# aask1357/hilcodec

Hardware: AMD Instinct MI355X
Metric: audio-seconds/sec (xRT) encode+RVQ+decode, 24 kHz batch=256 (higher is better)
Workload: dtype f32

## Files before the change

hilcodec_amd/csrc/resblock_cfg.h:

```cpp
#pragma once
#include <stdlib.h>

#include <atomic>
#include <type_traits>

#include "gemm_core.h"

using namespace hilc;

namespace {

constexpr int DWS = 12;

#ifndef HILC_RES_SHARE2_0
#define HILC_RES_SHARE2_0 0.61
#endif
#ifndef HILC_RES_SHARE3_0
#define HILC_RES_SHARE3_0 0.44
#define HILC_RES_SHARE3_1 0.31
#endif
template <int C, bool STREAM, bool SCARRY_ = false, int NB_ = 1, bool W8_ = false, int DR_ = 0, bool POST_ = false, bool SPEC0_ = false>
struct Cfg {
  static constexpr bool POST = POST_;
  static constexpr bool SPEC0 = SPEC0_;
  static_assert(!SPEC0_ || (C == 64 && (!STREAM || SCARRY_) && !W8_ && DR_ >= 0), "stage-0 input phase: the C = 64 encoder stage in the carry form (four waves, 128-column tiles)");
  static_assert(!POST_ || ((!STREAM || SCARRY_) && DR_ <= 0 && C <= 192 && !W8_), "closing conv: the carry form of a narrow stage (offline, or a hop's runs of whole streams)");
  static constexpr int NB = NB_;
  static constexpr int DR = DR_ > 0 ? DR_ : 0;
  static constexpr int UR = DR_ < 0 ? -DR_ : 0;
  static_assert(DR_ <= 0 || (((DR_ == 2 || DR_ == 4) && (!STREAM || SCARRY_) && C <= 192) || ((!STREAM || SCARRY_) && DR_ == 5 && C == 256) || (!SCARRY_ && DR_ == 8 && C == 512)),
                "down-sampling phase: carry form, r = 2 / 4 (C <= 192) or the wide encoder stages (C = 256: r = 5, offline and the hop's 32-column carry form; C = 512: r = 8, offline and a hop's whole-stream tiles)");
  static constexpr int DCAR = DR_ <= 0 ? 0 : (DR_ == 5 ? 12 : (DR_ == 8 ? 8 : 4));
  static_assert(DR_ >= 0 || ((DR_ == -8 && C >= 512) || (DR_ == -5 && C == 384) || ((DR_ == -4 || DR_ == -2) && C <= 192 && (!STREAM || SCARRY_))),
                "up-sampling phase: 32-column tiles (r = 8: whole streams, or the offline carry form), the C = 384 stage (r = 5) or the carry form (r = 4 / 2)");
  static constexpr int CH = C;
  static constexpr int CB = C / 32;
  static constexpr bool NARROW = C >= 256;
  static constexpr bool N32 = STREAM && SCARRY_ && NARROW;
  static_assert(!N32 || C == 256 || C == 384, "32-column carry form: the C = 256 / C = 384 stages of a hop");
  static constexpr int NCOL = NARROW ? ((C >= 512 || N32) ? 32 : 64) : 128;
  static constexpr int XS = NCOL + ((!STREAM || SCARRY_) ? 8 * NB_ + 2 * DCAR + (POST_ ? 4 : 0) : 0);
  static constexpr bool CARRYMODE = !STREAM || SCARRY_;
  static constexpr int HALO = CARRYMODE ? 0 : ((NARROW && C >= 512) ? 0 : 8);
  static constexpr int TO = NCOL - HALO;
  static constexpr int NW = (N32 && C == 384) ? 12 : ((C >= 192 || W8_) ? 8 : 4);
  static constexpr int NT = 64 * NW;
  static constexpr int RH = NW / (NCOL / 32);
  static constexpr int CBW = CB / RH;
  static constexpr int RPI = 256 / NCOL;
  static constexpr int RSTEP = RPI * NW;
  static constexpr int RW = C / RSTEP;
#ifndef HILC_RES_RB
#define HILC_RES_RB 4
#endif
  static constexpr int RB = HILC_RES_RB;
#ifdef HILC_RES_KP
  static constexpr int KP = HILC_RES_KP;
  static constexpr int DEPTH = HILC_RES_DEPTH;
#else
  static constexpr int KP = C >= 96 ? 4 : 8;
  static constexpr int DEPTH = C >= 256 ? 4 : (C == 128 ? (STREAM ? 2 : 3) : 2);
#endif
#ifndef HILC_RES_MINW
#define HILC_RES_MINW 2
#endif
  static constexpr int MINW = NW >= 8 ? NW / 4 : HILC_RES_MINW;
  static_assert(NW % (NCOL / 32) == 0 && CB % RH == 0 && RW % RB == 0 && C % RSTEP == 0, "tile split");
  static_assert(NB_ >= 1 && NB_ <= 3 && (NB_ == 1 || CARRYMODE || (NARROW && C >= 512)), "a chain needs carries or whole-stream tiles");
};

struct ResBlk {
  const float* w1t;
  const float* dw1_w;
  const float* dw1_b;
  const float* w2t;
  const float* dw2_w;
  const float* dw2_b;
  const float* hist1;
  const float* hist2;
  float* hist1_out;
  float* hist2_out;
  float pre_scale, out_scale;
};

struct ResUp {
  const float* xin;
  const float* tr_w;
  const float* w_lo;
  const float* w_hi;
  const float* bias;
  const float* hist;
  float* hist_out;
  float in_scale;
};

struct ResDown {
  const float* w_lo;
  const float* w_hi;
  const float* dw_w;
  const float* dw_b;
  const float* hist;
  float* hist_out;
  const float* res;
  float* y;
  float in_scale;
};

struct ResPost {
  const float* w;
  const float* bias;
  float* wav;
  const float* hist;
  float* hist_out;
  float in_scale, out_scale;
  int do_tanh;
};

struct ResSpec0 {
  const float* wav;
  const float* dft;
  const float* nyq;
  const float* pw;
  const float* bias;
  const float* pre_w;
  const float* pre_b;
  const float* hist;
  int hist_len;
  float pre_in_scale, mean, stdv, out_scale;
  int normalize;
};

constexpr int POST_CLASSES = 8;

constexpr int MAXBLK = 3;
constexpr int DDS = 12;

struct ResArgs {
  const float* x;
  ResBlk blk[MAXBLK];
  int nblk;
  ResDown dn;
  ResUp up;
  ResPost post;
  ResSpec0 spec;
  long run_tiles;
  float* y;
  int T, tiles;
  int classes;
  unsigned cum[5];
  long total_tiles;
  int B;
  unsigned div_magic, div_shift;
  int* sched;
  unsigned long long* dbg;
};

#ifdef HILC_DEBUG_STAMPS
unsigned long long* g_dbg = nullptr;
#endif

}
```

hilcodec_amd/csrc/resblock_gemm.h:

```cpp
#pragma once
#include "resblock_cfg.h"

namespace {

typedef const __attribute__((address_space(1))) float* gptr_t;
typedef __attribute__((address_space(3))) float* lptr_t;
typedef __attribute__((address_space(3))) f32x4* lvec_t;
typedef __attribute__((address_space(3))) f32x2* lvec2_t;

template <class K>
struct WeightPipe {
  static constexpr int CBW = K::CBW;
  static constexpr int DEPTH = K::DEPTH;
  static constexpr int KP = K::KP;
  static constexpr int WPS = KP * CBW / 4;
  static_assert(KP * CBW % 4 == 0 && 8 % KP == 0, "register set = whole 16-B words");
  float a[DEPTH][KP][CBW];
  __device__ __forceinline__ void load_word(gptr_t wset, int slot, int q, int lane) {
    typedef const __attribute__((address_space(1))) f32x4* gvec_t;
    const f32x4 v = *(gvec_t)(wset + q * 256 + lane * 4);
#pragma unroll
    for (int e = 0; e < 4; ++e) a[slot][(q * 4 + e) / CBW][(q * 4 + e) % CBW] = v[e];
  }
  __device__ __forceinline__ void prefetch(const float* __restrict__ wt, int lane) {
#pragma unroll
    for (int d = 0; d < DEPTH - 1; ++d)
#pragma unroll
      for (int q = 0; q < WPS; ++q) load_word((gptr_t)(wt + d * WPS * 256), d, q, lane);
  }
};


template <class K, bool ZERO = true>
__device__ __forceinline__ void gemm_phase(const float* __restrict__ wt, const float* X, f32x16 (&acc)[K::CBW],
                                           WeightPipe<K>& wp, int colblk, int lane) {
  constexpr int C = K::CH, XS = K::XS;
  constexpr int CBW = K::CBW;
  constexpr int DEPTH = WeightPipe<K>::DEPTH, KP = WeightPipe<K>::KP, WPS = WeightPipe<K>::WPS;
  constexpr int NSETS = C / 2 / KP;
  const int kh = lane >> 5, l31 = lane & 31;
  lptr_t xn = (lptr_t)(X + kh * XS + colblk * 32 + l31);
  float b[DEPTH][KP];
#pragma unroll
  for (int d = 0; d < DEPTH - 1; ++d) {
#pragma unroll
    for (int j = 0; j < KP; ++j) b[d][j] = xn[j * 2 * XS];
    xn += KP * 2 * XS;
    asm volatile("" : "+v"(xn));
  }
  constexpr int LD_EVERY = KP * CBW / WPS;
  const float* wn = wt + (DEPTH - 1) * WPS * 256;
#pragma unroll
  for (int s = 0; s < NSETS; ++s) {
    const int cur = s % DEPTH, nxt = (s + DEPTH - 1) % DEPTH;
    const int sn = s + DEPTH - 1;
    const bool more = sn < NSETS;
#pragma unroll
    for (int j = 0; j < KP; ++j) {
      if (more) b[nxt][j] = xn[j * 2 * XS];
#pragma unroll
      for (int i = 0; i < CBW; ++i) {
        const int n = j * CBW + i;
        if (more && n % LD_EVERY == 0) wp.load_word((gptr_t)wn, nxt, n / LD_EVERY, lane);
        if (ZERO && s == 0 && j == 0) {
#pragma unroll
          for (int r = 0; r < 16; ++r) acc[i][r] = 0.f;
        }
        acc[i] = __builtin_amdgcn_mfma_f32_32x32x2f32(wp.a[cur][j][i], b[cur][j], acc[i], 0, 0, 0);
      }
    }
    if (more) {
      xn += KP * 2 * XS;
      wn += WPS * 256;
      asm volatile("" : "+v"(xn), "+s"(wn));
    }
#pragma unroll
    for (int i = 0; i < CBW; ++i) asm volatile("" : "+v"(acc[i]) :: "memory");
  }
}

template <class K, bool ZERO = true>
__device__ __forceinline__ void gemm_phase_rolled(const float* __restrict__ wt, const float* X, f32x16 (&acc)[K::CBW],
                                                  WeightPipe<K>& wp, int colblk, int lane) {
  constexpr int C = K::CH, XS = K::XS;
  constexpr int CBW = K::CBW;
  constexpr int DEPTH = WeightPipe<K>::DEPTH, KP = WeightPipe<K>::KP, WPS = WeightPipe<K>::WPS;
  constexpr int NSETS = C / 2 / KP;
  static_assert(NSETS % DEPTH == 0 && NSETS >= 2 * DEPTH, "whole groups of register sets");
  constexpr int NG = NSETS / DEPTH;
  const int kh = lane >> 5, l31 = lane & 31;
  lptr_t xn = (lptr_t)(X + kh * XS + colblk * 32 + l31);
  float b[DEPTH][KP];
#pragma unroll
  for (int d = 0; d < DEPTH - 1; ++d) {
#pragma unroll
    for (int j = 0; j < KP; ++j) b[d][j] = xn[j * 2 * XS];
    xn += KP * 2 * XS;
    asm volatile("" : "+v"(xn));
  }
  constexpr int LD_EVERY = KP * CBW / WPS;
  const float* wn = wt + (DEPTH - 1) * WPS * 256;
  if constexpr (ZERO) {
#pragma unroll
    for (int i = 0; i < CBW; ++i)
#pragma unroll
      for (int r = 0; r < 16; ++r) acc[i][r] = 0.f;
  }
  auto one_set = [&](auto dc, bool more) {
    constexpr int cur = decltype(dc)::value, nxt = (cur + DEPTH - 1) % DEPTH;
#pragma unroll
    for (int j = 0; j < KP; ++j) {
      if (more) b[nxt][j] = xn[j * 2 * XS];
#pragma unroll
      for (int i = 0; i < CBW; ++i) {
        const int n = j * CBW + i;
        if (more && n % LD_EVERY == 0) wp.load_word((gptr_t)wn, nxt, n / LD_EVERY, lane);
        acc[i] = __builtin_amdgcn_mfma_f32_32x32x2f32(wp.a[cur][j][i], b[cur][j], acc[i], 0, 0, 0);
      }
    }
    if (more) {
      xn += KP * 2 * XS;
      wn += WPS * 256;
      asm volatile("" : "+v"(xn), "+s"(wn));
    }
#pragma unroll
    for (int i = 0; i < CBW; ++i) asm volatile("" : "+v"(acc[i]) :: "memory");
  };
  auto group = [&](bool last) {
    one_set(std::integral_constant<int, 0>{}, true);
    if constexpr (DEPTH > 1) one_set(std::integral_constant<int, 1>{}, !last);
    if constexpr (DEPTH > 2) one_set(std::integral_constant<int, 2>{}, !last);
    if constexpr (DEPTH > 3) one_set(std::integral_constant<int, 3>{}, !last);
    static_assert(DEPTH <= 4, "group body");
  };
#pragma nounroll
  for (int g = 0; g < NG - 1; ++g) group(false);
  group(true);
}

template <class K>
__device__ __forceinline__ void acc_to_x(const f32x16 (&acc)[K::CBW], float* X, int rowblk0, int colblk, int lane) {
  constexpr int XS = K::XS;
  lptr_t xb = (lptr_t)(X + (rowblk0 * 32 + 4 * (lane >> 5)) * XS + colblk * 32 + (lane & 31));
#pragma unroll
  for (int i = 0; i < K::CBW; ++i) {
#pragma unroll
    for (int r = 0; r < 16; ++r) xb[((r & 3) + 8 * (r >> 2)) * XS] = acc[i][r];
    xb += 32 * XS;
    asm volatile("" : "+v"(xb));
  }
}

__device__ __forceinline__ void lds_barrier() { asm volatile("s_waitcnt lgkmcnt(0)\n\ts_barrier" ::: "memory"); }

}
```

hilcodec_amd/csrc/resblock_kernel.h:

```cpp
#pragma once
#include "resblock_gemm.h"
#include "stream_gemm.h"

namespace {

struct Cols {
  long b;
  int t;
  int t_in;
  unsigned boff;
  unsigned hoff;
  int head, tail;
};
static_assert(sizeof(Cols) == 32, "no padding");

template <int C, bool STREAM, bool SCARRY = false, int NB = 1, bool W8 = false, int DRU = 0, bool POST = false, bool SPEC0 = false>
__global__ __launch_bounds__((Cfg<C, STREAM, SCARRY, NB, W8, DRU, POST, SPEC0>::NT), (Cfg<C, STREAM, SCARRY, NB, W8, DRU, POST, SPEC0>::MINW)) void resblock_kernel(ResArgs a) {
  using K = Cfg<C, STREAM, SCARRY, NB, W8, DRU, POST, SPEC0>;
  constexpr int DR = K::DR, UR = K::UR;
  using Pipe = WeightPipe<K>;
  constexpr int CBW = K::CBW, NW = K::NW, NT = K::NT, RW = K::RW, RB = K::RB, XS = K::XS, TO = K::TO, RSTEP = K::RSTEP;
  __shared__ __attribute__((aligned(16))) float Xbuf[4 + C * XS];
  constexpr bool DW_RELOAD = NB > 1 && K::NARROW && (4 + C * XS + NB * C * DWS) * 4 > 156 * 1024;
  __shared__ __attribute__((aligned(16))) float DW[(DW_RELOAD ? 1 : NB) * C * DWS];
// ... 106 lines not shown
          if (C % NT == 0 || m < C) {
#pragma unroll
            for (int w4 = 0; w4 < DWS / 4; ++w4)
              *reinterpret_cast<f32x4*>(&DW[(q * C + m) * DWS + 4 * w4]) =
                  f32x4{tv[q][it][4 * w4], tv[q][it][4 * w4 + 1], tv[q][it][4 * w4 + 2], tv[q][it][4 * w4 + 3]};
          }
        }
      }
    }
    }
  }
  if constexpr (DR > 0 && !DWIDE) {
    constexpr int RND = (2 * C + NT - 1) / NT;
    float tw[RND][2 * DR + 1];
#pragma unroll
    for (int it = 0; it < RND; ++it) {
      const int m = tid + it * NT;
      const int mc = ((2 * C) % NT == 0 || m < 2 * C) ? m : 2 * C - 1;
#pragma unroll
      for (int j = 0; j < 2 * DR; ++j) tw[it][j] = a.dn.dw_w[mc * 2 * DR + j];
      tw[it][2 * DR] = a.dn.dw_b[mc];
    }
#pragma unroll
    for (int it = 0; it < RND; ++it) {
      const int m = tid + it * NT;
      if ((2 * C) % NT == 0 || m < 2 * C) {
#pragma unroll
        for (int j = 0; j < DDS; ++j) DWD[m * DDS + j] = j < 2 * DR ? tw[it][j] : (j == 8 ? tw[it][2 * DR] : 0.f);
      }
    }
  }
  if (tid < 4) Xbuf[tid] = 0.f;
  const int rsub = wave * K::RPI + (K::RPI > 1 ? lane / (K::NCOL / 4) : 0);
  const int c4 = (lane & (K::NCOL / 4 - 1)) * 4;
  [[maybe_unused]] const unsigned row_b = (unsigned)T * 4u;
  [[maybe_unused]] const bool one_head = STREAM && !K::NARROW && T >= K::NCOL;

  auto columns_of = [&](long tile) -> Cols {
    Cols s;
    s.boff = 0; s.hoff = 0; s.head = false; s.tail = false;
    if constexpr (STREAM) {
      const int flat = (int)tile * TO - K::HALO + c4;
      s.t_in = flat >= 0 && flat < a.B * T;
      const unsigned ub = s.t_in ? __umulhi((unsigned)flat, a.div_magic) >> a.div_shift : 0u;
      s.b = ub;
      s.t = s.t_in ? flat - (int)ub * T : 0;
      s.boff = (ub * (unsigned)(C * T) + (unsigned)s.t) * 4u;
      s.hoff = ub * (unsigned)(C * 4);
      s.head = s.t_in && s.t == 0;
      s.tail = s.t_in && c4 >= K::HALO && s.t == T - 4;
    } else {
      s.b = tile / a.tiles;
      s.t = (int)(tile - s.b * a.tiles) * TO + c4;
      s.t_in = s.t >= 0 && s.t < T;
    }
    return s;
  };
  auto xrow = [&](const Cols& s, int m) -> const f32x4* {
    if constexpr (STREAM)
      return reinterpret_cast<const f32x4*>(reinterpret_cast<const char*>(a.x) + (s.boff + (unsigned)m * row_b));
    else
      return reinterpret_cast<const f32x4*>(a.x + s.b * (long)C * T + (long)m * T + (s.t_in ? s.t : 0));
  };
  auto yrow = [&](const Cols& s, int m) -> f32x4* {
    if constexpr (STREAM)
      return reinterpret_cast<f32x4*>(reinterpret_cast<char*>(a.y) + (s.boff + (unsigned)m * row_b));
    else
      return reinterpret_cast<f32x4*>(a.y + s.b * (long)C * T + (long)m * T + s.t);
  };

  [[maybe_unused]] const float* hb0 = a.x;
  [[maybe_unused]] const float* hb1 = a.x;
  [[maybe_unused]] bool hv0 = false, hv1 = false;
  [[maybe_unused]] int blk_off = 0;
  Cols cs;
  const bool lane0 = c4 == 0, lane_last = c4 == K::NCOL - 4;
  auto prev_base = [&](int which) -> lptr_t {
    if constexpr (!K::CARRYMODE) return (lptr_t)(X + rsub * XS + c4 - 4);
    else return lane0 ? (lptr_t)(X + rsub * XS + K::NCOL + which * 4 + blk_off) : (lptr_t)(X + rsub * XS + c4 - 4);
  };
  auto prevs_of = [&](lptr_t pb, int m0, int which, f32x4 (&prev)[K::RB]) {
    if constexpr (!STREAM) {
#pragma unroll
      for (int i = 0; i < K::RB; ++i) prev[i] = *(lvec_t)(pb + i * RSTEP * XS);
    } else {
      bool staged = false;
      if constexpr (!K::NARROW) staged = one_head;
      if (staged) {
#pragma unroll
        for (int i = 0; i < K::RB; ++i) {
          const lptr_t pa = cs.head ? (lptr_t)(HS + (which * C + m0 + RSTEP * i) * 4) : pb + i * RSTEP * XS;
          prev[i] = *(lvec_t)pa;
        }
      } else {
        f32x4 hv[K::RB];
#pragma unroll
        for (int i = 0; i < K::RB; ++i)
          hv[i] = *reinterpret_cast<const f32x4*>((which ? hb1 : hb0) + ((which ? hv1 : hv0) ? cs.hoff + (unsigned)(m0 + RSTEP * i) * 4u : 0u));
#pragma unroll
        for (int i = 0; i < K::RB; ++i) {
          const f32x4 own = *(lvec_t)(pb + i * RSTEP * XS);
#pragma unroll
          for (int e = 0; e < 4; ++e) prev[i][e] = cs.head ? ((which ? hv1 : hv0) ? hv[i][e] : 0.f) : own[e];
        }
      }
    }
  };
  auto carry_out = [&](lptr_t xp, int which, const f32x4 (&cur)[K::RB]) {
    if constexpr (K::CARRYMODE) {
      if (lane_last) {
#pragma unroll
        for (int i = 0; i < K::RB; ++i) *(lvec_t)(xp + i * RSTEP * XS + 4 + which * 4 + blk_off) = cur[i];
      }
    }
  };

  float touch = 0.f;
  constexpr int LPR = K::NCOL / 32;
#ifdef HILC_RES_NO_UTOUCH
  constexpr bool UTOUCH = false;
#else
  constexpr bool UTOUCH = !STREAM && UR > 0 && !K::NARROW && (K::NCOL / (UR > 0 ? UR : 1)) % 32 == 0;
#endif
  constexpr int LPRU = UTOUCH ? K::NCOL / UR / 32 : 1;
  constexpr int NTOUCH = STREAM ? 1 : (UTOUCH ? (2 * C * LPRU + NT - 1) / NT : (C * LPR + NT - 1) / NT);
  float tv[NTOUCH];
#pragma unroll
  for (int i = 0; i < NTOUCH; ++i) tv[i] = 0.f;
  __shared__ long s_next;
  long run0 = blockIdx.x, run1 = a.total_tiles;
  long tile = blockIdx.x;
  if constexpr (K::CARRYMODE) {
    if (a.classes > 1) {
      const unsigned P = gridDim.x / (unsigned)a.classes, u = blockIdx.x % P, c = blockIdx.x / P;
      const long s0 = (long)u * a.total_tiles / P, len = (long)(u + 1) * a.total_tiles / P - s0;
      run0 = s0 + ((len * (long)a.cum[c]) >> 16);
      run1 = s0 + ((len * (long)a.cum[c + 1]) >> 16);
    } else if (a.run_tiles > 0) {
      run0 = (long)blockIdx.x * a.run_tiles;
      run1 = run0 + a.run_tiles < a.total_tiles ? run0 + a.run_tiles : a.total_tiles;
    } else {
      run0 = (long)blockIdx.x * a.total_tiles / gridDim.x;
      run1 = ((long)blockIdx.x + 1) * a.total_tiles / gridDim.x;
    }
    const bool mid = STREAM ? (run0 * TO) % T != 0 : run0 % a.tiles != 0;
    tile = (mid && run0 < run1) ? run0 - 1 : run0;
  }
  cs = columns_of(tile < run1 ? tile : 0);
  f32x4 xr[RW];
  if (UR == 0 && !SPEC0 && tile < run1) {
#pragma unroll
    for (int i = 0; i < RW; ++i) xr[i] = *xrow(cs, rsub + RSTEP * i);
  }
  lds_barrier();
  while (tile < run1) {
    const bool warm = K::CARRYMODE && tile < run0;
    constexpr bool TICKETS = !K::CARRYMODE && K::NW == 4;
    if constexpr (K::CARRYMODE && !STREAM) {
      if (tile % a.tiles == 0) {
        constexpr int NSLOT = 2 * NB + K::DCAR / 2 + (POST ? 1 : 0);
        for (int e = tid; e < NSLOT * C; e += NT)
          *reinterpret_cast<f32x4*>(X + (e / NSLOT) * XS + K::NCOL + (e % NSLOT) * 4) = f32x4{0.f, 0.f, 0.f, 0.f};
      }
    }
    if constexpr (!K::CARRYMODE) {
      if (TICKETS && a.sched != nullptr && tid == 0) s_next = (long)gridDim.x + atomicAdd(a.sched, 1);
    }
#if defined(HILC_DEBUG_WAVE_STAMPS)
    if (a.dbg != nullptr) {
      if (ws_base != nullptr && lane == 0) ws_base[(WS_MAXB - 1) * 3 + 1] = (unsigned long long)ws_k;
      ws_base = a.dbg + ((tile * NW + wave) * (long)WS_MAXB) * 3;
      if (lane == 0) { ws_base[(WS_MAXB - 1) * 3] = blockIdx.x; ws_base[(WS_MAXB - 1) * 3 + 2] = __builtin_amdgcn_s_memtime(); }
    }
    ws_k = 0;
#elif defined(HILC_DEBUG_STAMPS)
    stamp_tile = tile;
#endif
    STAMP(0);
    long next_tile = K::CARRYMODE ? tile + 1 : tile + gridDim.x;
    if constexpr (UR > 0) {
      const ResUp& up = a.up;
      const int Tin = T / UR;
      const int q0 = cs.t / UR, p0 = cs.t - q0 * UR;
      f32x16 acc[CBW];
#pragma unroll
      for (int i = 0; i < CBW; ++i)
#pragma unroll
        for (int r = 0; r < 16; ++r) acc[i][r] = 0.f;
#pragma nounroll
      for (int h = 0; h < 2; ++h) {
        const float* wu = (h ? up.w_hi : up.w_lo) + (long)wclass * (C * C / K::RH);
        asm volatile("" : "+s"(wu));
        {
          constexpr int UB = RW % 6 == 0 ? 6 : RB;
          constexpr bool UEXP = UR == 5;
          lptr_t xp = (lptr_t)(X + rsub * XS + c4);
          const bool has_prev = cs.t_in && q0 >= 1;
          [[maybe_unused]] const bool has_next = cs.t_in && q0 + 1 < Tin;
#pragma unroll
          for (int i0 = 0; i0 < RW; i0 += UB) {
            float xc[UB], xq[UB];
            [[maybe_unused]] float xn[UB];
            f32x4 wa[UB];
            [[maybe_unused]] f32x4 wb[UB];
#pragma unroll
            for (int i = 0; i < UB; ++i) {
              const int k = h * C + rsub + RSTEP * (i0 + i);
              const long row = (long)cs.b * (2 * C) + k;
              const float* xi = up.xin + (cs.t_in ? row * Tin + q0 : 0);
              xc[i] = xi[0];
              const float* pp = has_prev ? xi - 1 : (up.hist != nullptr && cs.t_in ? up.hist + row : xi);
              xq[i] = pp[0];
              if constexpr (UR == 2) {
                xn[i] = xi[cs.t_in ? 1 : 0];
                wa[i] = *reinterpret_cast<const f32x4*>(up.tr_w + k * 4);
              } else if constexpr (UEXP) {
                xn[i] = xi[has_next ? 1 : 0];
                const float* tw = up.tr_w + ((long)k * UR + p0) * 8;
                wa[i] = *reinterpret_cast<const f32x4*>(tw);
                wb[i] = *reinterpret_cast<const f32x4*>(tw + 4);
              } else {
                wa[i] = *reinterpret_cast<const f32x4*>(up.tr_w + k * (2 * UR) + p0);
                wb[i] = *reinterpret_cast<const f32x4*>(up.tr_w + k * (2 * UR) + UR + p0);
              }
            }
#pragma unroll
            for (int i = 0; i < UB; ++i) {
              const float a1 = prologue(xc[i], up.in_scale, 1);
              const float a0 = has_prev ? prologue(xq[i], up.in_scale, 1) : (up.hist != nullptr ? xq[i] : 0.f);
              f32x4 u;
              float a_last = a1;
              if constexpr (UR == 2) {
                const float a2 = prologue(xn[i], up.in_scale, 1);
                u[0] = fmaf(wa[i].x, a1, wa[i].z * a0);
                u[1] = fmaf(wa[i].y, a1, wa[i].w * a0);
                u[2] = fmaf(wa[i].x, a2, wa[i].z * a1);
                u[3] = fmaf(wa[i].y, a2, wa[i].w * a1);
                a_last = a2;
              } else if constexpr (UEXP) {
                const float a2 = has_next ? prologue(xn[i], up.in_scale, 1) : 0.f;
#pragma unroll
                for (int e = 0; e < 4; ++e) {
                  const bool nx = p0 + e >= UR;
                  u[e] = fmaf(wa[i][e], nx ? a2 : a1, wb[i][e] * (nx ? a1 : a0));
                }
                a_last = p0 + 3 >= UR ? a2 : a1;
              } else {
#pragma unroll
                for (int e = 0; e < 4; ++e) u[e] = fmaf(wa[i][e], a1, wb[i][e] * a0);
              }
              *(lvec_t)(xp + i * RSTEP * XS) = zero_unless(cs.t_in, u);
              if constexpr (STREAM) {
                if (cs.tail && !warm && up.hist_out != nullptr)
                  up.hist_out[(long)cs.b * (2 * C) + h * C + rsub + RSTEP * (i0 + i)] = a_last;
              }
            }
            xp += UB * RSTEP * XS;
            asm volatile("" : "+v"(xp));
            __builtin_amdgcn_sched_barrier(0);
          }
        }
        Pipe wp;
        wp.prefetch(wu, lane);
        lds_barrier();
        if constexpr (K::NARROW) gemm_phase_rolled<K, false>(wu, X, acc, wp, colblk, lane);
        else gemm_phase<K, false>(wu, X, acc, wp, colblk, lane);
        lds_barrier();
      }
      acc_to_x<K>(acc, X, rowblk0, colblk, lane);
      lds_barrier();
      {
        lptr_t xp = (lptr_t)(X + rsub * XS + c4);
#pragma unroll
        for (int i = 0; i < RW; ++i) {
          const float bv = up.bias != nullptr ? up.bias[rsub + RSTEP * i] : 0.f;
          f32x4 v = *(lvec_t)(xp + i * RSTEP * XS);
#pragma unroll
          for (int e = 0; e < 4; ++e) v[e] = up.bias != nullptr ? __fadd_rn(v[e], bv) : v[e];
          xr[i] = v;
        }
      }
      lds_barrier();
    }
    if constexpr (SPEC0) {
      const ResSpec0& sp = a.spec;
      constexpr int N = 64, NBIN = 33, SROWS = 40, KP0 = 4, DEPTH0 = 2;
      [[maybe_unused]] int split = K::NCOL;
      if constexpr (STREAM) {
        const int F0 = (int)tile * TO;
        const unsigned bA = __umulhi((unsigned)F0, a.div_magic) >> a.div_shift;
        const int tA0 = F0 - (int)bA * T;
        const int nxt = T - tA0;
        split = nxt < K::NCOL ? nxt : K::NCOL;
        const int lenA = (N - 1) + split;
        for (int i = tid; i < 2 * (N - 1) + K::NCOL; i += NT) {
          const bool second = i >= lenA;
          const unsigned b = bA + (second ? 1u : 0u);
          const int t = second ? i - lenA - (N - 1) : tA0 - (N - 1) + i;
          float v = 0.f;
          if (b < (unsigned)a.B) {
            if (t >= 0) v = sp.wav[(long)b * T + t];
            else if (sp.hist != nullptr && t >= -sp.hist_len) v = sp.hist[(long)b * sp.hist_len + sp.hist_len + t];
          }
          SEG[i] = v;
          SEGS[i] = v * sp.pre_in_scale;
        }
        for (int i = tid; i < (SROWS - NBIN) * 128; i += NT) X[(NBIN + (i >> 7)) * XS + (i & 127)] = 0.f;
      } else {
      const int f0 = cs.t - c4;
      {
        const int s0 = f0 - (N - 1);
        const float* wb = sp.wav + cs.b * (long)T;
        for (int i = tid; i < 127 + N; i += NT) {
          const int t = s0 + i;
          const float v = (t >= 0 && t < T) ? wb[t] : 0.f;
          SEG[i] = v;
          SEGS[i] = v * sp.pre_in_scale;
        }
        for (int i = tid; i < (SROWS - NBIN) * 128; i += NT) X[(NBIN + (i >> 7)) * XS + (i & 127)] = 0.f;
      }
      }
      lds_barrier();
      const int kh = lane >> 5, col = colblk * 32 + (lane & 31);
      const int colx = col + ((STREAM && col >= split) ? N - 1 : 0);
      f32x16 acc[CBW];
      {
        int off[8];
#pragma unroll
        for (int p = 0; p < 8; ++p) off[p] = colx + 2 * p + kh;
        auto bop = [&](int P) -> float { return SEG[off[P & 7] + 16 * (P >> 3)]; };
        stream_gemm<CBW, KP0, DEPTH0, N / 2 / KP0>(sp.dft, acc, lane, bop);
      }
      float nyq_im = 0.f;
#pragma unroll 8
      for (int k = 0; k < N; ++k) nyq_im = fmaf(sp.nyq[k], SEG[colx + k], nyq_im);
      const SpecFinish finish = SpecFinish::make(sp.mean, sp.stdv, sp.normalize);
#pragma unroll
      for (int i = 0; i < CBW; ++i) {
#pragma unroll
        for (int r = 0; r < 16; r += 2) {
          const int row = i * 32 + acc_row(r, lane);
          if (i == 0 && r == 0) {
            if (kh == 0) {
              X[0 * XS + col] = finish(acc[0][0], 0.f);
              X[(N / 2) * XS + col] = finish(acc[0][1], nyq_im);
            } else {
              X[(row >> 1) * XS + col] = finish(acc[0][0], acc[0][1]);
            }
          } else {
            X[(row >> 1) * XS + col] = finish(acc[i][r], acc[i][r + 1]);
          }
        }
      }
      lds_barrier();
      {
        const float* sl = X + kh * XS + col;
        auto bop = [&](int P) -> float { return sl[2 * P * XS]; };
        stream_gemm<CBW, KP0, DEPTH0, SROWS / 2 / KP0>(sp.pw, acc, lane, bop);
      }
      lds_barrier();
      acc_to_x<K>(acc, X, rowblk0, colblk, lane);
      lds_barrier();
      {
        lptr_t xp = (lptr_t)(X + rsub * XS + c4);
        float sm[8];
        const int c4x = c4 + ((STREAM && c4 >= split) ? N - 1 : 0);
#pragma unroll
        for (int j = 0; j < 8; ++j) sm[j] = SEGS[c4x + j + N - 5];
#pragma unroll
        for (int i = 0; i < RW; ++i) {
          const int m = rsub + RSTEP * i;
          const float bv = sp.bias != nullptr ? sp.bias[m] : 0.f;
          const float pb = sp.pre_b != nullptr ? sp.pre_b[m] : 0.f;
          float w5[5];
#pragma unroll
          for (int j = 0; j < 5; ++j) w5[j] = sp.pre_w[m * 5 + j];
          f32x4 v = *(lvec_t)(xp + i * RSTEP * XS);
#pragma unroll
          for (int e = 0; e < 4; ++e) {
            float acc5 = 0.f;
#pragma unroll
            for (int j = 0; j < 5; ++j) acc5 = fmaf(w5[j], sm[e + j], acc5);
            const float rr = sp.pre_b != nullptr ? __fadd_rn(acc5, pb) : acc5;
            float t = v[e];
            if (sp.bias != nullptr) t = __fadd_rn(t, bv);
            t = __fmul_rn(t, sp.out_scale);
            v[e] = __fadd_rn(t, rr);
          }
          xr[i] = v;
          if (i % 2 == 1) __builtin_amdgcn_sched_barrier(0);
        }
      }
      lds_barrier();
    }
#pragma nounroll
    for (int blk = 0; blk < nblk; ++blk) {
    const ResBlk& bp = a.blk[NB == 1 ? 0 : blk];
    const bool final_blk = NB == 1 || blk == nblk - 1;
    const bool last_blk = DR == 0 && !POST && final_blk;
    [[maybe_unused]] const bool post_blk = POST && final_blk;
    Cols cn = cs;
    bool have_next = false;
    if constexpr (NB > 1) blk_off = 8 * blk;
    const float* const DWb = DW + ((NB == 1 || DW_RELOAD) ? 0 : blk * C * DWS);
    if constexpr (DW_RELOAD) load_taps(bp, DW);
    if constexpr (STREAM) {
      hb0 = bp.hist1 != nullptr ? bp.hist1 : a.x;
      hb1 = bp.hist2 != nullptr ? bp.hist2 : a.x;
      hv0 = bp.hist1 != nullptr;
      hv1 = bp.hist2 != nullptr;
    }
    const float* w1t = bp.w1t + (long)wclass * (C * C / K::RH);
    const float* w2t = bp.w2t + (long)wclass * (C * C / K::RH);
    asm volatile("" : "+s"(w1t), "+s"(w2t));
    [[maybe_unused]] f32x4 hstage[(STREAM && !K::NARROW) ? (2 * C + NT - 1) / NT : 1];
    [[maybe_unused]] bool stage_hs = false;
    if constexpr (STREAM && !K::NARROW) {
      if (one_head) {
        const int first = (int)tile * TO - K::HALO, last = first + K::NCOL - 1;
        const unsigned bh = __umulhi((unsigned)last, a.div_magic) >> a.div_shift;
        const int hcol = (int)bh * T;
        stage_hs = hcol >= first && (int)bh < a.B;
        if (stage_hs) {
#pragma unroll
          for (int q = 0; q < (2 * C + NT - 1) / NT; ++q) {
            const int e = tid + q * NT;
            const int which = e >= C ? 1 : 0, m = e - which * C;
            f32x4 v = {0.f, 0.f, 0.f, 0.f};
            if (e < 2 * C && (which ? hv1 : hv0)) v = *reinterpret_cast<const f32x4*>((which ? hb1 : hb0) + bh * (unsigned)(C * 4) + (unsigned)m * 4u);
            hstage[q] = v;
          }
        }
      }
    }
    Pipe wp;
    wp.prefetch(w1t, lane);
    {
      lptr_t xp = (lptr_t)(X + rsub * XS + c4);
#pragma unroll
      for (int i0 = 0; i0 < RW; i0 += RB) {
#pragma unroll
        for (int i = 0; i < RB; ++i)
          *(lvec_t)(xp + i * RSTEP * XS) = prologue4v(zero_unless(cs.t_in, xr[i0 + i]), bp.pre_scale, 1);
        xp += RB * RSTEP * XS;
        asm volatile("" : "+v"(xp));
      }
    }
#pragma unroll
    for (int i = 0; i < NTOUCH; ++i) touch += tv[i];
    if constexpr (STREAM && !K::NARROW) {
      if (stage_hs) {
#pragma unroll
        for (int q = 0; q < (2 * C + NT - 1) / NT; ++q) {
          const int e = tid + q * NT;
          if (e < 2 * C) *reinterpret_cast<f32x4*>(&HS[e * 4]) = hstage[q];
        }
      }
    }
    lds_barrier();
    STAMP(1);
    if (TICKETS && a.sched != nullptr) next_tile = s_next;

    f32x16 acc[CBW];
    if constexpr (K::NARROW) gemm_phase_rolled<K>(w1t, X, acc, wp, colblk, lane);
    else gemm_phase<K>(w1t, X, acc, wp, colblk, lane);
    lds_barrier();
    STAMP(2);
    acc_to_x<K>(acc, X, rowblk0, colblk, lane);
    lds_barrier();
    STAMP(3);

    wp.prefetch(w2t, lane);
    lptr_t xp3 = (lptr_t)(X + rsub * XS + c4);
    lptr_t pb3 = prev_base(0);
#pragma unroll
    for (int i0 = 0; i0 < RW; i0 += RB) {
      f32x4 cur[RB], prev[RB], wa[RB];
      f32x2 wb[RB];
#pragma unroll
      for (int i = 0; i < RB; ++i) {
        const int m = rsub + RSTEP * (i0 + i);
        const lptr_t row = xp3 + i * RSTEP * XS;
        cur[i] = *(lvec_t)(row);
        wa[i] = *reinterpret_cast<const f32x4*>(&DWb[m * DWS]);
        wb[i] = *reinterpret_cast<const f32x2*>(&DWb[m * DWS + 4]);
      }
      prevs_of(pb3, rsub + RSTEP * i0, 0, prev);
      carry_out(xp3, 0, cur);
      if constexpr (STREAM) {
        if (cs.tail && !warm && bp.hist1_out != nullptr) {
#pragma unroll
          for (int i = 0; i < RB; ++i)
            *reinterpret_cast<f32x4*>(bp.hist1_out + cs.hoff + (rsub + RSTEP * (i0 + i)) * 4) = cur[i];
        }
      }
      f32x4 o[RB];
#pragma unroll
      for (int i = 0; i < RB; ++i) {
        const float v[8] = {prev[i].x, prev[i].y, prev[i].z, prev[i].w, cur[i].x, cur[i].y, cur[i].z, cur[i].w};
        const float w[5] = {wa[i].x, wa[i].y, wa[i].z, wa[i].w, wb[i].x};
#pragma unroll
        for (int e = 0; e < 4; ++e) {
          float s = 0.f;
#pragma unroll
          for (int j = 0; j < 5; ++j) s = fmaf(w[j], v[e + j], s);
          o[i][e] = elu_fast(__fadd_rn(s, wb[i].y));
        }
      }
#pragma unroll
      for (int i = 0; i < RB; ++i)
        *(lvec_t)(xp3 + i * RSTEP * XS) = o[i];
      xp3 += RB * RSTEP * XS;
      pb3 += RB * RSTEP * XS;
      asm volatile("" : "+v"(xp3), "+v"(pb3));
      __builtin_amdgcn_sched_barrier(0);
    }
    lds_barrier();
    STAMP(4);

    if constexpr (K::NARROW) gemm_phase_rolled<K>(w2t, X, acc, wp, colblk, lane);
    else gemm_phase<K>(w2t, X, acc, wp, colblk, lane);
    have_next = next_tile < run1;
    if (last_blk) cn = columns_of(have_next ? next_tile : tile);
    if constexpr (!STREAM && UR == 0 && !SPEC0) {
      if (final_blk) {
      long nb;
      int nt0;
      if constexpr (STREAM) {
        const int nf0 = (int)(have_next ? next_tile : tile) * TO - K::HALO;
        const unsigned q = __umulhi((unsigned)(nf0 < 0 ? 0 : nf0), a.div_magic) >> a.div_shift;
        nb = q;
        nt0 = nf0 - (int)q * T;
      } else {
        const long nt = have_next ? next_tile : tile;
        nb = nt / a.tiles;
        nt0 = (int)(nt - nb * a.tiles) * TO;
      }
      const float* nx = a.x + nb * (long)C * T;
#pragma unroll
      for (int i = 0; i < NTOUCH; ++i) {
        int e = tid + NT * i;
        e = e < C * LPR ? e : C * LPR - 1;
        int tt = nt0 + (e % LPR) * 32;
        tt = tt < 0 ? 0 : (tt > T - 1 ? T - 1 : tt);
        tv[i] = nx[(long)(e / LPR) * T + tt];
      }
      }
    }
    if constexpr (UTOUCH) {
      if (final_blk) {
        const long nt = have_next ? next_tile : tile;
        const long nb = nt / a.tiles;
        const int Tin = T / UR;
        const int nq0 = (int)(nt - nb * a.tiles) * TO / UR;
        const float* nx = a.up.xin + nb * (long)(2 * C) * Tin;
#pragma unroll
        for (int i = 0; i < NTOUCH; ++i) {
          int e = tid + NT * i;
          e = e < 2 * C * LPRU ? e : 2 * C * LPRU - 1;
          int ff = nq0 + (e % LPRU) * 32;
          ff = ff > Tin - 1 ? Tin - 1 : ff;
          tv[i] = nx[(long)(e / LPRU) * Tin + ff];
        }
      }
    }
    lds_barrier();
    STAMP(5);
    acc_to_x<K>(acc, X, rowblk0, colblk, lane);
    lds_barrier();
    STAMP(6);

    const bool out_ok = !warm && (STREAM ? (c4 >= K::HALO && cs.t_in) : cs.t < T);
    lptr_t xp6 = (lptr_t)(X + rsub * XS + c4);
    lptr_t pb6 = prev_base(1);
#pragma unroll
    for (int i0 = 0; i0 < RW; i0 += RB) {
      f32x4 cur[RB], prev[RB], wc[RB];
      f32x2 wb[RB];
#pragma unroll
      for (int i = 0; i < RB; ++i) {
        const int m = rsub + RSTEP * (i0 + i);
        const lptr_t row = xp6 + i * RSTEP * XS;
        cur[i] = *(lvec_t)(row);
        wb[i] = *reinterpret_cast<const f32x2*>(&DWb[m * DWS + 6]);
        wc[i] = *reinterpret_cast<const f32x4*>(&DWb[m * DWS + 8]);
      }
      prevs_of(pb6, rsub + RSTEP * i0, 1, prev);
      carry_out(xp6, 1, cur);
      if constexpr (STREAM) {
        if (cs.tail && !warm && bp.hist2_out != nullptr) {
#pragma unroll
          for (int i = 0; i < RB; ++i)
            *reinterpret_cast<f32x4*>(bp.hist2_out + cs.hoff + (rsub + RSTEP * (i0 + i)) * 4) = cur[i];
        }
      }
#pragma unroll
      for (int i = 0; i < RB; ++i) {
        const int m = rsub + RSTEP * (i0 + i);
        const float v[8] = {prev[i].x, prev[i].y, prev[i].z, prev[i].w, cur[i].x, cur[i].y, cur[i].z, cur[i].w};
        const float w[5] = {wb[i].x, wb[i].y, wc[i].x, wc[i].y, wc[i].z};
        f32x4 o;
#pragma unroll
        for (int e = 0; e < 4; ++e) {
          float s = 0.f;
#pragma unroll
          for (int j = 0; j < 5; ++j) s = fmaf(w[j], v[e + j], s);
          s = __fmul_rn(__fadd_rn(s, wc[i].w), bp.out_scale);
          o[e] = __fadd_rn(s, xr[i0 + i][e]);
        }
        if constexpr (NB == 1 && DR == 0 && !POST) {
          if (out_ok) *yrow(cs, m) = o;
        } else {
          if (last_blk) {
            if (out_ok) *yrow(cs, m) = o;
          } else if (post_blk) {
            *(lvec_t)(xp6 + i * RSTEP * XS) = prologue4v(o, a.post.in_scale, 1);
          } else {
            xr[i0 + i] = o;
          }
        }
      }
      if (UR == 0 && !SPEC0 && last_blk && have_next) {
#pragma unroll
        for (int i = 0; i < RB; ++i) xr[i0 + i] = *xrow(cn, rsub + RSTEP * (i0 + i));
      }
      xp6 += RB * RSTEP * XS;
      pb6 += RB * RSTEP * XS;
      asm volatile("" : "+v"(xp6), "+v"(pb6));
      __builtin_amdgcn_sched_barrier(0);
    }
    STAMP(7);
    lds_barrier();
    if (last_blk) cs = cn;
    }
    if constexpr (POST) {
      const bool have_next = next_tile < run1;
      const Cols cn = columns_of(have_next ? next_tile : tile);
      constexpr int PSLOT = K::NCOL + 8 * NB;
      float part[4] = {0.f, 0.f, 0.f, 0.f};
      lptr_t xq = (lptr_t)(X + rsub * XS + c4);
      lptr_t pq = lane0 ? (lptr_t)(X + rsub * XS + PSLOT) : (lptr_t)(X + rsub * XS + c4 - 4);
      const float* wq = a.post.w + rsub * 5;
      [[maybe_unused]] bool any_head = false;
      [[maybe_unused]] const float* hq = a.post.w;
      [[maybe_unused]] float* hqo = nullptr;
      [[maybe_unused]] bool qtail = false;
      if constexpr (STREAM) {
        const int first = (int)tile * TO, last = first + K::NCOL - 1;
        const unsigned bl = __umulhi((unsigned)last, a.div_magic) >> a.div_shift;
        any_head = (int)bl * T >= first || first % T == 0;
        if (a.post.hist != nullptr) hq = a.post.hist + cs.hoff + rsub * 4;
        qtail = cs.tail && !warm && a.post.hist_out != nullptr;
        if (a.post.hist_out != nullptr) hqo = a.post.hist_out + cs.hoff + rsub * 4;
      }
#pragma nounroll
      for (int i0 = 0; i0 < RW; i0 += RB) {
        f32x4 cur[RB], prev[RB];
        float w[RB][5];
#pragma unroll
        for (int i = 0; i < RB; ++i) {
          cur[i] = *(lvec_t)(xq + i * RSTEP * XS);
          prev[i] = *(lvec_t)(pq + i * RSTEP * XS);
#pragma unroll
          for (int j = 0; j < 5; ++j) w[i][j] = wq[i * RSTEP * 5 + j];
        }
        wq += RB * RSTEP * 5;
        if constexpr (STREAM) {
          if (any_head) {
            f32x4 hv[RB];
#pragma unroll
            for (int i = 0; i < RB; ++i)
              hv[i] = a.post.hist != nullptr ? *reinterpret_cast<const f32x4*>(hq + i * RSTEP * 4) : f32x4{0.f, 0.f, 0.f, 0.f};
#pragma unroll
            for (int i = 0; i < RB; ++i)
#pragma unroll
              for (int e = 0; e < 4; ++e) prev[i][e] = cs.head ? hv[i][e] : prev[i][e];
          }
          if (qtail) {
#pragma unroll
            for (int i = 0; i < RB; ++i) *reinterpret_cast<f32x4*>(hqo + i * RSTEP * 4) = cur[i];
          }
          hq += a.post.hist != nullptr ? RB * RSTEP * 4 : 0;
          hqo += RB * RSTEP * 4;
        }
        if (lane_last) {
#pragma unroll
          for (int i = 0; i < RB; ++i) *(lvec_t)(xq + i * RSTEP * XS + 4 + 8 * NB) = cur[i];
        }
#pragma unroll
        for (int i = 0; i < RB; ++i) {
          const float v[8] = {prev[i].x, prev[i].y, prev[i].z, prev[i].w, cur[i].x, cur[i].y, cur[i].z, cur[i].w};
#pragma unroll
          for (int e = 0; e < 4; ++e)
#pragma unroll
            for (int j = 0; j < 5; ++j) part[e] = fmaf(w[i][j], v[e + j], part[e]);
        }
        xq += RB * RSTEP * XS;
        pq += RB * RSTEP * XS;
        asm volatile("" : "+v"(xq), "+v"(pq));
        __builtin_amdgcn_sched_barrier(0);
      }
      *reinterpret_cast<f32x4*>(&PR[rsub * K::NCOL + c4]) = f32x4{part[0], part[1], part[2], part[3]};
      lds_barrier();
      if (tid < K::NCOL) {
        float sacc = PR[tid];
#pragma unroll
        for (int q = 1; q < POST_CLASSES; ++q) sacc = __fadd_rn(sacc, PR[q * K::NCOL + tid]);
        if (a.post.bias != nullptr) sacc = __fadd_rn(sacc, a.post.bias[0]);
        sacc = __fmul_rn(sacc, a.post.out_scale);
        if (a.post.do_tanh) sacc = tanhf(sacc);
        if constexpr (STREAM) {
          const long flat = (long)tile * TO + tid;
          if (!warm && flat < (long)a.B * T) a.post.wav[flat] = sacc;
        } else {
          const int t = cs.t - c4 + tid;
          if (!warm && t < T) a.post.wav[cs.b * (long)T + t] = sacc;
        }
      }
      cs = cn;
    }
    if constexpr (DR > 0) {
      const ResDown& dn = a.dn;
      const bool have_next = next_tile < run1;
      const Cols cn = columns_of(have_next ? next_tile : tile);
      const float* wd0 = dn.w_lo + (long)wclass * (C * C / K::RH);
      const float* wd1 = dn.w_hi + (long)wclass * (C * C / K::RH);
      asm volatile("" : "+s"(wd0), "+s"(wd1));
      Pipe wp;
      wp.prefetch(wd0, lane);
      auto d0 = [&]() {
        lptr_t xp = (lptr_t)(X + rsub * XS + c4);
#pragma unroll
        for (int i0 = 0; i0 < RW; i0 += RB) {
#pragma unroll
          for (int i = 0; i < RB; ++i)
            *(lvec_t)(xp + i * RSTEP * XS) = prologue4v(zero_unless(cs.t_in, xr[i0 + i]), dn.in_scale, 1);
          xp += RB * RSTEP * XS;
          asm volatile("" : "+v"(xp));
        }
      };
      d0();
      if (!DWIDE && !SPEC0 && have_next) {
#pragma unroll
        for (int i = 0; i < RW; ++i) xr[i] = *xrow(cn, rsub + RSTEP * i);
      }
      lds_barrier();
      f32x16 acc0[CBW];
      [[maybe_unused]] f32x16 acc1[DWIDE ? 1 : CBW];
      if constexpr (K::NARROW) gemm_phase_rolled<K>(wd0, X, acc0, wp, colblk, lane);
      else gemm_phase<K>(wd0, X, acc0, wp, colblk, lane);
      if constexpr (!DWIDE) {
        wp.prefetch(wd1, lane);
        if constexpr (K::NARROW) gemm_phase_rolled<K>(wd1, X, acc1, wp, colblk, lane);
        else gemm_phase<K>(wd1, X, acc1, wp, colblk, lane);
      }
      const bool out_ok = !warm && (STREAM ? cs.t_in : cs.t < T);
      [[maybe_unused]] const bool out_ok_tile = !warm;
      const int To = T / DR;
#pragma unroll
      for (int h = 0; h < 2; ++h) {
        if constexpr (DWIDE) {
          if (h == 1) {
            lds_barrier();
            wp.prefetch(wd1, lane);
            d0();
            if (have_next) {
#pragma unroll
              for (int i = 0; i < RW; ++i) xr[i] = *xrow(cn, rsub + RSTEP * i);
            }
            lds_barrier();
            gemm_phase_rolled<K>(wd1, X, acc0, wp, colblk, lane);
          }
        }
        lds_barrier();
        if constexpr (DWIDE) acc_to_x<K>(acc0, X, rowblk0, colblk, lane);
        else acc_to_x<K>(h ? acc1 : acc0, X, rowblk0, colblk, lane);
        lds_barrier();
// ... 233 lines not shown
```

Before: 3531.

## Fuse transposed-conv upsampling into the GEMM operand fetch for C=192 r=4 stage

For the offline C=192 decoder stage with 4x upsampling, the per-tile input frames and the transposed-conv taps are staged compactly in LDS. The upsampled B-operand is then computed on the fly inside a new GEMM routine that runs both weight halves (lo/hi) as one pipelined loop. The next tile's input frames are prefetched into registers during the previous tile's epilogue. This is meant to remove the separate upsampling pass with its LDS write-out and the barrier between the two half-GEMMs. In exchange it adds extra ALU work per operand fetch and more register pressure.

```diff
diff --git a/hilcodec_amd/csrc/resblock_cfg.h b/hilcodec_amd/csrc/resblock_cfg.h
--- a/hilcodec_amd/csrc/resblock_cfg.h
+++ b/hilcodec_amd/csrc/resblock_cfg.h
@@ -28,6 +28,8 @@
   static constexpr int NB = NB_;
   static constexpr int DR = DR_ > 0 ? DR_ : 0;
   static constexpr int UR = DR_ < 0 ? -DR_ : 0;
+  static constexpr bool UOP = !STREAM && DR_ == -4 && C == 192;
+  static constexpr int UPASS = 1;
   static_assert(DR_ <= 0 || (((DR_ == 2 || DR_ == 4) && (!STREAM || SCARRY_) && C <= 192) || ((!STREAM || SCARRY_) && DR_ == 5 && C == 256) || (!SCARRY_ && DR_ == 8 && C == 512)),
                 "down-sampling phase: carry form, r = 2 / 4 (C <= 192) or the wide encoder stages (C = 256: r = 5, offline and the hop's 32-column carry form; C = 512: r = 8, offline and a hop's whole-stream tiles)");
   static constexpr int DCAR = DR_ <= 0 ? 0 : (DR_ == 5 ? 12 : (DR_ == 8 ? 8 : 4));
diff --git a/hilcodec_amd/csrc/resblock_gemm.h b/hilcodec_amd/csrc/resblock_gemm.h
--- a/hilcodec_amd/csrc/resblock_gemm.h
+++ b/hilcodec_amd/csrc/resblock_gemm.h
@@ -138,6 +138,70 @@
   group(true);
 }
 
+template <int R, int PSTR>
+struct UpOperand {
+  lptr_t ap, tp;
+  struct Raw { float a0, a1, w0, w1; };
+  __device__ __forceinline__ Raw fetch(int j) const { return Raw{ap[j * PSTR], ap[j * PSTR + 1], tp[j * PSTR], tp[j * PSTR + R]}; }
+  static __device__ __forceinline__ float value(const Raw& r) { return fmaf(r.w0, r.a1, __fmul_rn(r.w1, r.a0)); }
+  template <int KP>
+  __device__ __forceinline__ void advance() {
+    ap += KP * PSTR;
+    tp += KP * PSTR;
+    asm volatile("" : "+v"(ap), "+v"(tp));
+  }
+};
+
+template <class K, int NH, bool ZERO, class BOp>
+__device__ __forceinline__ void gemm_phase_op(const float* const (&wt)[NH], f32x16 (&acc)[K::CBW], WeightPipe<K>& wp, int lane, BOp& bop) {
+  constexpr int C = K::CH, CBW = K::CBW;
+  constexpr int DEPTH = WeightPipe<K>::DEPTH, KP = WeightPipe<K>::KP, WPS = WeightPipe<K>::WPS;
+  constexpr int HSETS = C / 2 / KP, NSETS = NH * HSETS;
+  static_assert(DEPTH - 1 <= HSETS && DEPTH <= NSETS, "the prefetched sets lie in the first matrix");
+  float b[DEPTH][KP];
+  typename BOp::Raw raw[KP];
+#pragma unroll
+  for (int d = 0; d < DEPTH - 1; ++d) {
+#pragma unroll
+    for (int j = 0; j < KP; ++j) b[d][j] = BOp::value(bop.fetch(j));
+    bop.template advance<KP>();
+  }
+#pragma unroll
+  for (int j = 0; j < KP; ++j) raw[j] = bop.fetch(j);
+  bop.template advance<KP>();
+  constexpr int LD_EVERY = KP * CBW / WPS;
+  const float* wn = wt[0] + (DEPTH - 1) * WPS * 256;
+#pragma unroll
+  for (int s = 0; s < NSETS; ++s) {
+    const int cur = s % DEPTH, nxt = (s + DEPTH - 1) % DEPTH;
+    const int sn = s + DEPTH - 1;
+    const bool more = sn < NSETS, more2 = sn + 1 < NSETS;
+#pragma unroll
+    for (int j = 0; j < KP; ++j) {
+      if (more) b[nxt][j] = BOp::value(raw[j]);
+      if (more2) raw[j] = bop.fetch(j);
+#pragma unroll
+      for (int i = 0; i < CBW; ++i) {
+        const int n = j * CBW + i;
+        if (more && n % LD_EVERY == 0) wp.load_word((gptr_t)wn, nxt, n / LD_EVERY, lane);
+        if (ZERO && s == 0 && j == 0) {
+#pragma unroll
+          for (int r = 0; r < 16; ++r) acc[i][r] = 0.f;
+        }
+        acc[i] = __builtin_amdgcn_mfma_f32_32x32x2f32(wp.a[cur][j][i], b[cur][j], acc[i], 0, 0, 0);
+      }
+    }
+    if (more2) bop.template advance<KP>();
+    if (more) {
+      if ((sn + 1) % HSETS == 0 && (sn + 1) / HSETS < NH) wn = wt[(sn + 1) / HSETS];
+      else wn += WPS * 256;
+      asm volatile("" : "+s"(wn));
+    }
+#pragma unroll
+    for (int i = 0; i < CBW; ++i) asm volatile("" : "+v"(acc[i]) :: "memory");
+  }
+}
+
 template <class K>
 __device__ __forceinline__ void acc_to_x(const f32x16 (&acc)[K::CBW], float* X, int rowblk0, int colblk, int lane) {
   constexpr int XS = K::XS;
diff --git a/hilcodec_amd/csrc/resblock_kernel.h b/hilcodec_amd/csrc/resblock_kernel.h
--- a/hilcodec_amd/csrc/resblock_kernel.h
+++ b/hilcodec_amd/csrc/resblock_kernel.h
@@ -282,6 +282,46 @@
 #pragma unroll
     for (int i = 0; i < RW; ++i) xr[i] = *xrow(cs, rsub + RSTEP * i);
   }
+  constexpr int UFPR = K::UOP ? K::NCOL / UR : 1, USRI = NT / UFPR;
+  constexpr int UNIT = K::UOP ? 2 * C / USRI : 1;
+  constexpr int UTW = K::UOP ? 2 * UR / 4 : 1, UNTW = K::UOP ? (2 * C * UTW + NT - 1) / NT : 1;
+  [[maybe_unused]] float ufv[UNIT];
+  [[maybe_unused]] float upv = 0.f;
+  [[maybe_unused]] f32x4 utw[UNTW];
+  constexpr int UPARTS = RW / RB;
+  static_assert(!K::UOP || UNIT % UPARTS == 0, "whole parts");
+  [[maybe_unused]] const float* uxh = a.up.xin;
+  [[maybe_unused]] unsigned ufo = 0;
+  [[maybe_unused]] long upo = 0;
+  [[maybe_unused]] auto uop_aim = [&](long nt) {
+    const long nb = nt / a.tiles;
+    const int Tin = T / (UR > 0 ? UR : 1);
+    const int qf = __builtin_amdgcn_readfirstlane((int)(nt - nb * a.tiles)) * (TO / (UR > 0 ? UR : 1));
+    uxh = a.up.xin + (long)__builtin_amdgcn_readfirstlane((int)nb) * (2 * C) * Tin + qf;
+    const int fl = tid % UFPR, fr = tid / UFPR;
+    ufo = qf + fl < Tin ? (unsigned)(fr * Tin + fl) : 0u;
+    upo = (tid < 2 * C && qf > 0) ? (long)tid * Tin - 1 : 0L;
+  };
+  [[maybe_unused]] auto uop_load = [&](int part) {
+    const int Tin = T / (UR > 0 ? UR : 1);
+#pragma unroll
+    for (int i = part * (UNIT / UPARTS); i < (part + 1) * (UNIT / UPARTS); ++i) ufv[i] = (uxh + (long)(i * USRI) * Tin)[ufo];
+    if (part == 0) upv = uxh[upo];
+  };
+  if constexpr (K::UOP) {
+#pragma unroll
+    for (int i = 0; i < UNIT; ++i) ufv[i] = 0.f;
+#pragma unroll
+    for (int i = 0; i < UNTW; ++i) {
+      const int e = tid + i * NT;
+      utw[i] = *reinterpret_cast<const f32x4*>(a.up.tr_w + ((2 * C * UTW) % NT == 0 || e < 2 * C * UTW ? e : 0) * 4);
+    }
+    if (tile < run1) {
+      uop_aim(tile);
+#pragma unroll
+      for (int part = 0; part < UPARTS; ++part) uop_load(part);
+    }
+  }
   lds_barrier();
   while (tile < run1) {
     const bool warm = K::CARRYMODE && tile < run0;
@@ -311,12 +351,54 @@
     if constexpr (UR > 0) {
       const ResUp& up = a.up;
       const int Tin = T / UR;
-      const int q0 = cs.t / UR, p0 = cs.t - q0 * UR;
+      [[maybe_unused]] const int q0 = cs.t / UR, p0 = cs.t - q0 * UR;
       f32x16 acc[CBW];
 #pragma unroll
       for (int i = 0; i < CBW; ++i)
 #pragma unroll
         for (int r = 0; r < 16; ++r) acc[i][r] = 0.f;
+      if constexpr (K::UOP) {
+        constexpr int FPR = UFPR, SRI = USRI, NIT = UNIT, TW = UTW, NTW = UNTW;
+        constexpr int ZS = FPR + 2, TP = FPR + 4, RL = TP + 2 * UR;
+        static_assert(2 * RL <= K::NCOL && RL % 4 == 0 && XS % 4 == 0, "two staged rows in front of a tile row's carry slots, tap words 16-B aligned");
+        static_assert(NT % FPR == 0 && SRI % 2 == 0 && (2 * C) % SRI == 0 && NIT % 8 == 0 && 2 * C <= NT, "whole rounds of row pairs");
+        const int t0 = __builtin_amdgcn_readfirstlane(cs.t - c4);
+        const float* wus[2] = {up.w_lo + (long)wclass * (C * C / K::RH), up.w_hi + (long)wclass * (C * C / K::RH)};
+        asm volatile("" : "+s"(wus[0]), "+s"(wus[1]));
+        Pipe wp;
+        wp.prefetch(wus[0], lane);
+        {
+          const int fl = tid % FPR, fr = tid / FPR;
+          lptr_t fp = (lptr_t)(X + (fr >> 1) * XS + (fr & 1) * RL + 1 + fl);
+#pragma unroll
+          for (int i0 = 0; i0 < NIT; i0 += 8) {
+#pragma unroll
+            for (int i = 0; i < 8; ++i) fp[i * (SRI / 2) * XS] = prologue(ufv[i0 + i], up.in_scale, 1);
+            fp += 8 * (SRI / 2) * XS;
+            asm volatile("" : "+v"(fp));
+          }
+          if (tid < 2 * C) {
+            lptr_t rp = (lptr_t)(X + (tid >> 1) * XS + (tid & 1) * RL);
+            rp[0] = t0 > 0 ? prologue(upv, up.in_scale, 1) : 0.f;
+            rp[ZS] = 0.f;
+            rp[ZS + 1] = 0.f;
+          }
+#pragma unroll
+          for (int i = 0; i < NTW; ++i) {
+            const int e = tid + i * NT, k = e / TW;
+            if ((2 * C * TW) % NT == 0 || e < 2 * C * TW) *(lvec_t)(X + (k >> 1) * XS + (k & 1) * RL + TP + 4 * (e % TW)) = utw[i];
+          }
+        }
+        lds_barrier();
+        {
+          const int kh = lane >> 5, col = colblk * 32 + (lane & 31);
+          UpOperand<UR, XS> bop;
+          bop.ap = (lptr_t)(X + kh * RL + (t0 + col < T ? col / UR : ZS));
+          bop.tp = (lptr_t)(X + kh * RL + TP + col % UR);
+          gemm_phase_op<K, 2, true>(wus, acc, wp, lane, bop);
+        }
+        lds_barrier();
+      } else {
 #pragma nounroll
       for (int h = 0; h < 2; ++h) {
         const float* wu = (h ? up.w_hi : up.w_lo) + (long)wclass * (C * C / K::RH);
@@ -396,6 +478,7 @@
         if constexpr (K::NARROW) gemm_phase_rolled<K, false>(wu, X, acc, wp, colblk, lane);
         else gemm_phase<K, false>(wu, X, acc, wp, colblk, lane);
         lds_barrier();
+      }
       }
       acc_to_x<K>(acc, X, rowblk0, colblk, lane);
       lds_barrier();
@@ -694,6 +777,9 @@
         }
       }
     }
+    if constexpr (K::UOP) {
+      if (final_blk && have_next) uop_aim(next_tile);
+    }
     lds_barrier();
     STAMP(5);
     acc_to_x<K>(acc, X, rowblk0, colblk, lane);
@@ -753,6 +839,9 @@
       if (UR == 0 && !SPEC0 && last_blk && have_next) {
 #pragma unroll
         for (int i = 0; i < RB; ++i) xr[i0 + i] = *xrow(cn, rsub + RSTEP * (i0 + i));
+      }
+      if constexpr (K::UOP) {
+        if (final_blk && have_next) uop_load(i0 / RB);
       }
       xp6 += RB * RSTEP * XS;
       pb6 += RB * RSTEP * XS;
```

After: 3539 (median of 6 runs). About the same (+0.2%).
